# bertaveira/mojosplat

Hardware: AMD Instinct MI355X
Metric: frames/sec at 1M Gaussians 1920x1080 fwd; achieved HBM GB/s vs peak (higher is better)
Workload: dtype f32

## Files before the change

### mojosplat_amd/csrc/binning.hip

```cpp
#include <hip/hip_fp16.h>
#include <stdlib.h>
#include <string.h>

#include <algorithm>
#include <atomic>
#include <mutex>
#include <type_traits>
#include <vector>

#include "project_device.hpp"

#ifdef MS_DIAG
__device__ unsigned long long *g_diag_bin = nullptr;
#define MS_BIN_STAMP(k, j) do { if (g_diag_bin && threadIdx.x == 0 && blockIdx.x < 1024) g_diag_bin[((k) * 1024 + blockIdx.x) * 8 + (j)] = __builtin_amdgcn_s_memrealtime(); } while (0)
#else
#define MS_BIN_STAMP(k, j) do { } while (0)
#endif

namespace {

#ifndef MS_CHUNK
#define MS_CHUNK 2048
#endif
#ifndef MS_PH_WAVES
// ... 450 lines not shown
        unsigned long long bal[kSub];
        bool live[kSub];
        float p0[kSub], p1[kSub], p2[kSub], s0[kSub], s1[kSub], s2_[kSub];
#pragma unroll
        for (int k = 0; k < kSub; ++k) {
            const int64_t i = base + (int64_t)k * kHistThreads + threadIdx.x;
            live[k] = i < i1 && (!blocks || s_blk[(min(i, i1 - 1) >> block_shift) - blk0]);
            const int64_t j = live[k] ? i : i0;
            if constexpr (PREPARED) {
                const float4 r = cull[j];
                p0[k] = r.x; p1[k] = r.y; p2[k] = r.z; s0[k] = r.w; s1[k] = 0.f; s2_[k] = 0.f;
            } else {
                p0[k] = means3d[3 * j]; p1[k] = means3d[3 * j + 1]; p2[k] = means3d[3 * j + 2];
                s0[k] = scales[3 * j]; s1[k] = scales[3 * j + 1]; s2_[k] = scales[3 * j + 2];
            }
        }
#pragma unroll
        for (int k = 0; k < kSub; ++k) {
            keep[k] = false;
            {
                const float mx = V[0] * p0[k] + V[1] * p1[k] + V[2] * p2[k] + V[3];
                const float my = V[4] * p0[k] + V[5] * p1[k] + V[6] * p2[k] + V[7];
                const float z = V[8] * p0[k] + V[9] * p1[k] + V[10] * p2[k] + V[11];
                if (live[k] && !(z < P.near_plane || z > P.far_plane)) {
                    float sm = s0[k];
                    if constexpr (!PREPARED) {
                        sm = fmaxf(s0[k], fmaxf(s1[k], s2_[k]));
                        if (P.scales_are_log) sm = __expf(sm);
                    }
                    const float rz = __builtin_amdgcn_rcpf(z);
                    const float u = fminf(P.lim_x_pos, fmaxf(-P.lim_x_neg, mx * rz)), v = fminf(P.lim_y_pos, fmaxf(-P.lim_y_neg, my * rz));
                    const float s2 = lam * sm * sm;
                    const float fxz = P.fx * rz, fyz = P.fy * rz;
                    const float rx = 3.33f * __builtin_amdgcn_sqrtf(fxz * fxz * (1.0f + u * u) * s2 + P.eps2d) * 1.001f + 2.0f;
                    const float ry = 3.33f * __builtin_amdgcn_sqrtf(fyz * fyz * (1.0f + v * v) * s2 + P.eps2d) * 1.001f + 2.0f;
                    const float xs = P.fx * mx * rz + P.cx, ys = P.fy * my * rz + P.cy;
                    keep[k] = !(ys + ry < y_lo || ys - ry > y_hi || xs + rx < 0.f || xs - rx > P.W);
                }
            }
            bal[k] = __ballot(keep[k]);
        }
        uint32_t *sw = s_w[round & 1];
        ++round;
        if (lane == 0) {
#pragma unroll
            for (int k = 0; k < kSub; ++k) sw[k * 16 + w] = (uint32_t)__popcll(bal[k]);
        }
        __syncthreads();
#pragma unroll
        for (int k = 0; k < kSub; ++k) {
            uint32_t incl = lane < 16 ? sw[k * 16 + lane] : 0u;
#pragma unroll
            for (int d = 1; d < 16; d <<= 1) {
                const uint32_t o = (uint32_t)__shfl_up((int)incl, d);
                if (lane >= d) incl += o;
            }
            const int wu = __builtin_amdgcn_readfirstlane(w);
            const uint32_t total = (uint32_t)__builtin_amdgcn_readlane((int)incl, 15);
            const uint32_t before = written + (wu > 0 ? (uint32_t)__builtin_amdgcn_readlane((int)incl, wu - 1) : 0u);
            if (keep[k])
                seg[before + __builtin_amdgcn_mbcnt_hi((unsigned)(bal[k] >> 32), __builtin_amdgcn_mbcnt_lo((unsigned)bal[k], 0u))] =
                    (int32_t)(base + (int64_t)k * kHistThreads + threadIdx.x);
            written += total;
        }
    }
    if (threadIdx.x == 0) seg_count[blockIdx.x] = (int32_t)written;
    MS_BIN_STAMP(4, 2);
#ifdef MS_DIAG
    if (g_diag_bin && threadIdx.x == 0 && blockIdx.x < 1024) g_diag_bin[(4 * 1024 + blockIdx.x) * 8 + 3] = written;
#endif
}

template <bool PACK, int LEAN, bool CUT = false>
__global__ __launch_bounds__(kHistThreads, MS_PH_WAVES) void k_project_hist(
    int64_t N, const float *__restrict__ means3d, const float *__restrict__ scales,
    const float *__restrict__ quats, const float *__restrict__ opacities, const float *__restrict__ viewmat,
    ms::ProjParams P, Grid g, int64_t chunk, float *__restrict__ means2d, float *__restrict__ conics,
    float *__restrict__ depths, int32_t *__restrict__ radii, uint32_t *__restrict__ hist,
    uint32_t *__restrict__ wg_on_grid, unsigned long long *__restrict__ masks,
    const void *__restrict__ colors, int color_f16, float4 *__restrict__ rec, Candidates cand,
    LeanRec *__restrict__ lean, uint32_t *__restrict__ wg_depth, const uint32_t *__restrict__ tau,
    uint32_t *__restrict__ wg_far, uint32_t *__restrict__ has_far, uint32_t cut_stamp, LeanRec *__restrict__ near_recs,
    int keep_arrays, int64_t near_cap, unsigned int big_q_off, unsigned int big_q_cap,
    uint32_t *__restrict__ tile_total, unsigned long long *__restrict__ zero_flag, unsigned long long zero_stamp) {
    extern __shared__ uint32_t s_cnt[];
    const int T_local = (g.row_end - g.row_begin) * g.tw;
    unsigned int &s_on_grid = s_cnt[T_local];
    __shared__ unsigned int s_big_n;
    if (threadIdx.x == 0) s_big_n = 0;
    const BigQ bigq{reinterpret_cast<uint32_t *>(reinterpret_cast<char *>(s_cnt) + big_q_off), &s_big_n, big_q_cap};
    MS_BIN_STAMP(0, 0);
    __shared__ unsigned int s_near_n;
    __shared__ unsigned int s_next_slice;
    if (threadIdx.x == 0) { s_near_n = 0; s_next_slice = 0; }
    uint32_t *s_tau = s_cnt + T_local + 4;
    unsigned char *s_farflag = reinterpret_cast<unsigned char *>(s_tau + T_local);
    uint32_t far_pairs = 0;
    static_assert(!CUT || LEAN == 2, "depth-cut frames keep 12-byte box records");
    if constexpr (CUT)
        for (int t = threadIdx.x; t < T_local; t += kHistThreads) { s_tau[t] = tau[g.row_begin * g.tw + t]; s_farflag[t] = 0; }
    for (int t = threadIdx.x; t < T_local; t += kHistThreads) s_cnt[t] = 0;
    if (threadIdx.x == 0) { s_on_grid = 0; s_cnt[T_local + 1] = 0xffffffffu; s_cnt[T_local + 2] = 0u; s_cnt[T_local + 3] = 0u; }
    uint32_t dmin = 0xffffffffu, dmax = 0u;
    if (tile_total && blockIdx.x == 0) {
        for (int t = threadIdx.x; t < kClaimGroups * T_local; t += kHistThreads) __hip_atomic_store(&tile_total[t], 0u, __ATOMIC_RELAXED, __HIP_MEMORY_SCOPE_AGENT);
        asm volatile("s_waitcnt vmcnt(0)" ::: "memory");
    }
    __syncthreads();
    if (tile_total && blockIdx.x == 0 && threadIdx.x == 0)
        __hip_atomic_store(zero_flag, zero_stamp, __ATOMIC_RELEASE, __HIP_MEMORY_SCOPE_AGENT);
    __shared__ uint32_t s_pref[kMaxG + 1];
    CandMap map{s_pref};
    const int wg = chunk_of_block(blockIdx.x, gridDim.x);
    (void)chunk;
    int64_t i1 = N;
    if (cand.ids) {
        map.build(cand);
        i1 = (int64_t)s_pref[cand.n_segs];
    }
    const Deal deal(i1, wg, (int)gridDim.x);
    const uint32_t lane_u = threadIdx.x & 63u;
    auto count_plain = [&](int t, int64_t, int) __attribute__((always_inline)) { atomicAdd(&s_cnt[t], 1u); };
    auto count_cut = [&](int t, int64_t, int, uint32_t db) __attribute__((always_inline)) {
        if (db <= s_tau[t]) { atomicAdd(&s_cnt[t], 1u); dmin = min(dmin, db); dmax = max(dmax, db); }
        else { ++far_pairs; s_farflag[t] = 1; }
    };
    constexpr bool kTickets = kDeal == 64 && MS_PH_TICKETS != 0;
    const int n_slices = deal.iters * (kHistThreads / kDeal);
    for (int it = 0;; ++it) {
        int64_t base;
        if constexpr (kTickets) {
            int k = 0;
            if (lane_u == 0) k = (int)atomicAdd(&s_next_slice, 1u);
            k = __builtin_amdgcn_readfirstlane(k);
            if (k >= n_slices) break;
            base = ((int64_t)k * (int)gridDim.x + wg) * kDeal;
        } else {
            if (it >= deal.iters) break;
            base = deal.base(it);
        }
        const int64_t j = base + lane_u;
        int x0 = 0, x1 = 0, y0 = 0, y1 = 0, n = 0, edges = 0, gi = 0;
        bool on_grid = false;
        unsigned long long mask = ~0ull;
        uint32_t dbits_of_step = 0u;
        bool rec_pending = false;
        int64_t rec_b0 = 0;
        uint32_t rec_src = 0u;
        float rec_m0 = 0.f, rec_m1 = 0.f, rec_c0 = 0.f, rec_c1 = 0.f, rec_c2 = 0.f;
        auto write_record = [&](int64_t b0, uint32_t rec_src, float m0, float m1, float c0, float c1, float c2) __attribute__((always_inline)) {
            const float *opac_b = opacities ? opacities + b0 : nullptr;
            float col[3];
            if (color_f16) {
                const __half *c = reinterpret_cast<const __half *>(colors) + 3 * b0;
                col[0] = __half2float(c[3 * rec_src]); col[1] = __half2float(c[3 * rec_src + 1]); col[2] = __half2float(c[3 * rec_src + 2]);
            } else {
                const float *c = reinterpret_cast<const float *>(colors) + 3 * b0;
                const ms::F3 c3 = ms::ld_f32x3(c, rec_src);
                col[0] = c3.x; col[1] = c3.y; col[2] = c3.z;
            }
            const ms::RasterRecord r = ms::make_raster_record(m0, m1, c0, c1, c2, ms::ld_f32(opac_b, rec_src, 1, 0), col[0], col[1], col[2]);
            char *rb = reinterpret_cast<char *>(rec + 3 * base) + 48u * lane_u;
            *reinterpret_cast<float4 *>(rb) = r.a;
            *reinterpret_cast<float4 *>(rb + 16) = r.b;
            *reinterpret_cast<float4 *>(rb + 32) = r.c;
        };
        if (j < i1) {
            const bool gather = cand.ids != nullptr;
            const uint32_t src = gather ? (uint32_t)map.gaussian(cand, j) : lane_u;
            const int64_t b0 = gather ? 0 : base;
            const float *opac_b = opacities ? opacities + b0 : nullptr;
            const int64_t i = j;
            gi = (int)i;
            const ms::ProjOut o = ms::project_one<uint32_t, CUT>(src, means3d + 3 * b0, scales + 3 * b0, quats + 4 * b0, opac_b, viewmat, P);
            bool arrays = LEAN == 0;
            if constexpr (LEAN != 0) arrays = keep_arrays != 0;
            if (arrays) {
                reinterpret_cast<float2 *>(means2d)[i] = make_float2(o.m0, o.m1);
                conics[3 * i] = o.c0;
                conics[3 * i + 1] = o.c1;
                conics[3 * i + 2] = o.c2;
                depths[i] = o.d;
                reinterpret_cast<int2 *>(radii)[i] = make_int2(o.r0, o.r1);
            }
            if (rec && o.r0 > 0 && o.r1 > 0) {
                if constexpr (CUT) {
                    rec_pending = true;
                    rec_b0 = b0; rec_src = src;
                    rec_m0 = o.m0; rec_m1 = o.m1; rec_c0 = o.c0; rec_c1 = o.c1; rec_c2 = o.c2;
                } else {
                    write_record(b0, src, o.m0, o.m1, o.c0, o.c1, o.c2);
                }
            }
            if (o.r0 > 0 && o.r1 > 0) {
                on_grid = bin_box<PACK>(make_float2(o.m0, o.m1), make_int2(o.r0, o.r1), g, x0, x1, y0, y1, edges);
                n = (x1 - x0) * (y1 - y0);
                if (masks) {
                    if (LEAN == 2 && n > 32) mask = ~0ull;
                    else
                    if (PACK && n <= 16 && n > 0)
                        mask = clip_cells(reach_mask(o.m0, o.m1, o.c0, o.c1, o.c2, ms::ld_f32(opac_b, src, 1, 0), 2 * x0, 2 * x1,
                                                     2 * y0, 2 * y1, g.ts >> 1), edges, x1 - x0, y1 - y0);
                    else
                        mask = reach_mask(o.m0, o.m1, o.c0, o.c1, o.c2, ms::ld_f32(opac_b, src, 1, 0), x0, x1, y0, y1, g.ts);
                    if constexpr (LEAN != 2)
                        *reinterpret_cast<unsigned long long *>(reinterpret_cast<char *>(masks + base) + 8u * lane_u) = mask;
                }
            }
            dbits_of_step = __float_as_uint(o.d);
            if constexpr (LEAN != 0) {
                if (n > 0 && !CUT) { dmin = min(dmin, __float_as_uint(o.d)); dmax = max(dmax, __float_as_uint(o.d)); }
            }
            if constexpr (LEAN == 2 && !CUT) {
                uint32_t *q = reinterpret_cast<uint32_t *>(reinterpret_cast<char *>(reinterpret_cast<Lean12 *>(lean) + base) + 12u * lane_u);
                const uint32_t box = n > 0 ? ((uint32_t)x0 | ((uint32_t)y0 << 8) | ((uint32_t)(x1 - x0) << 16) | ((uint32_t)(y1 - y0) << 24)) : 0u;
                q[0] = box; q[1] = __float_as_uint(o.d); q[2] = (uint32_t)mask;
            }
            if constexpr (LEAN == 1)
                *reinterpret_cast<uint4 *>(reinterpret_cast<char *>(lean + base) + 16u * lane_u) = make_uint4((uint32_t)x0 | ((uint32_t)y0 << 16), (uint32_t)x1 | ((uint32_t)y1 << 16),
                                                                __float_as_uint(o.d), (uint32_t)n | ((uint32_t)edges << 28));
        }
        count_on_grid(on_grid, &s_on_grid);
        if constexpr (CUT) {
            uint32_t near32 = 0u;
            if (n > 0 && n <= kCoopThreshold) {
                const int w = x1 - x0;
                const float inv_w = __builtin_amdgcn_rcpf((float)w);
                unsigned int m = (unsigned int)mask & (n >= 32 ? 0xffffffffu : ((1u << n) - 1u));
                while (m) {
                    const int k = __ffs((int)m) - 1;
                    m &= m - 1;
                    const int r = (int)(((float)k + 0.5f) * inv_w);
                    const int t = (y0 + r - g.row_begin) * g.tw + x0 + (k - r * w);
                    if (dbits_of_step <= s_tau[t]) {
                        atomicAdd(&s_cnt[t], 1u);
                        near32 |= 1u << k;
                    } else {
                        ++far_pairs;
                        s_farflag[t] = 1;
                    }
                }
                if (near32) { dmin = min(dmin, dbits_of_step); dmax = max(dmax, dbits_of_step); }
            }
            walk_boxes<PACK>(gi, x0, x1, y0, y1, n > kCoopThreshold ? n : 0, edges, g, mask, count_cut, dbits_of_step, &bigq);
            const bool keep = near32 != 0u || n > kCoopThreshold;
            if (rec_pending && keep) write_record(rec_b0, rec_src, rec_m0, rec_m1, rec_c0, rec_c1, rec_c2);
            const unsigned long long kb = __ballot(keep);
            if (kb) {
                const int lane = threadIdx.x & 63;
                unsigned int wbase = 0;
                if (lane == 0) wbase = atomicAdd(&s_near_n, (unsigned int)__popcll(kb));
                wbase = (unsigned int)__builtin_amdgcn_readfirstlane((int)wbase);
                if (keep) {
                    const unsigned int pos = wbase + (unsigned int)__popcll(kb & ((1ull << lane) - 1ull));
                    const uint32_t box = (uint32_t)x0 | ((uint32_t)y0 << 8) | ((uint32_t)(x1 - x0) << 16) | ((uint32_t)(y1 - y0) << 24);
                    reinterpret_cast<uint4 *>(near_recs)[(int64_t)wg * near_cap + pos] = make_uint4(box, (uint32_t)gi, dbits_of_step, near32);
                }
            }
        } else {
            walk_boxes<PACK>(gi, x0, x1, y0, y1, n, edges, g, mask, count_plain, &bigq);
        }
    }
    if constexpr (CUT) drain_big_boxes<PACK, true>(bigq, g, count_cut);
    else drain_big_boxes<PACK, false>(bigq, g, count_plain);
    if constexpr (CUT) {
        {
#pragma unroll
            for (int d = 32; d > 0; d >>= 1) far_pairs += (uint32_t)__shfl_xor((int)far_pairs, d);
            if ((threadIdx.x & 63) == 0 && far_pairs) atomicAdd(&s_cnt[T_local + 3], far_pairs);
        }
    }
    if constexpr (LEAN != 0) {
        if (wg_depth) {
#pragma unroll
            for (int d = 32; d > 0; d >>= 1) {
                dmin = min(dmin, (uint32_t)__shfl_xor((int)dmin, d));
                dmax = max(dmax, (uint32_t)__shfl_xor((int)dmax, d));
            }
            if ((threadIdx.x & 63) == 0) { atomicMin(&s_cnt[T_local + 1], dmin); atomicMax(&s_cnt[T_local + 2], dmax); }
        }
    }
    MS_BIN_STAMP(0, 1);
    if (tile_total && threadIdx.x == 0) {
        while (__hip_atomic_load(zero_flag, __ATOMIC_ACQUIRE, __HIP_MEMORY_SCOPE_AGENT) != zero_stamp) __builtin_amdgcn_s_sleep(2);
    }
    __syncthreads();
    MS_BIN_STAMP(0, 2);
    uint32_t *row = hist + (size_t)wg * T_local;
    if (tile_total) {
        for (int t = threadIdx.x; t < T_local; t += kHistThreads) {
            const uint32_t c = s_cnt[t];
            row[t] = c ? __hip_atomic_fetch_add(&tile_total[(size_t)((blockIdx.x & 7) >> kClaimShift) * T_local + t], c, __ATOMIC_RELAXED, __HIP_MEMORY_SCOPE_AGENT) : 0u;
        }
    } else
    for (int t = threadIdx.x; t < T_local; t += kHistThreads) row[t] = s_cnt[t];
    if (threadIdx.x == 0) wg_on_grid[wg] = s_on_grid;
    if (threadIdx.x == 0 && blockIdx.x == 0) wg_on_grid[kMaxG] = 0;
    if constexpr (LEAN != 0) {
        if (wg_depth && threadIdx.x == 0) { wg_depth[2 * blockIdx.x] = s_cnt[T_local + 1]; wg_depth[2 * blockIdx.x + 1] = s_cnt[T_local + 2]; }
    }
    if constexpr (CUT) {
        {
            if (threadIdx.x == 0) { wg_far[wg] = s_cnt[T_local + 3]; wg_far[kMaxG + wg] = s_near_n; }
            for (int t = threadIdx.x; t < T_local; t += kHistThreads)
                if (s_farflag[t]) has_far[g.row_begin * g.tw + t] = cut_stamp;
        }
    }
    MS_BIN_STAMP(0, 3);
}

__global__ __launch_bounds__(kHistThreads) void k_isect_hist(
    int64_t N, const float *__restrict__ means2d, const int32_t *__restrict__ radii, Grid g,
    int64_t chunk, uint32_t *__restrict__ hist, int32_t *__restrict__ tiles_per_gauss,
    uint32_t *__restrict__ wg_on_grid) {
    extern __shared__ uint32_t s_cnt[];
    const int T_local = (g.row_end - g.row_begin) * g.tw;
    unsigned int &s_on_grid = s_cnt[T_local];
    for (int t = threadIdx.x; t < T_local; t += kHistThreads) s_cnt[t] = 0;
    if (threadIdx.x == 0) s_on_grid = 0;
    __syncthreads();
    const int wg = chunk_of_block(blockIdx.x, gridDim.x);
    (void)chunk;
    for_each_isect<false>(0, N, means2d, radii, nullptr, g, tiles_per_gauss, &s_on_grid, Candidates{nullptr, nullptr, 0, 0},
                   (int)gridDim.x, [&](int t, int64_t, int) { atomicAdd(&s_cnt[t], 1u); });
    __syncthreads();
    uint32_t *row = hist + (size_t)wg * T_local;
    for (int t = threadIdx.x; t < T_local; t += kHistThreads) row[t] = s_cnt[t];
    if (threadIdx.x == 0) wg_on_grid[wg] = s_on_grid;
    if (threadIdx.x == 0 && blockIdx.x == 0) wg_on_grid[kMaxG] = 0;
}

__device__ __forceinline__ int redo_signature(const Grid &g) { return (int)(0x80000000u | ((unsigned)g.tw & 0x7fffu) | (((unsigned)g.th & 0xffffu) << 15)); }

struct ScanTotalArgs {
    Grid g;
    const uint32_t *tile_count;
    int32_t *tile_ranges, *medium_list, *large_list, *xl_list;
    const uint32_t *wg_on_grid;
    int G;
    int32_t *redo_flag, *redo_count;
    int band_only;
    int64_t *info, *info_mirror;
    int32_t *order;
// ... 835 lines not shown
    const uint64_t k = src[start + e];
    flatten_ids[start + e] = (int32_t)(uint32_t)k;
    if (isect_ids) isect_ids[start + e] = ((int64_t)tile << 32) | (int64_t)(k >> 32);
}

__global__ __launch_bounds__(256) void k_offset_encode(int64_t M, const int64_t *__restrict__ ids,
                                                       int T, int32_t *__restrict__ offsets) {
    const int64_t idx = (int64_t)blockIdx.x * 256 + threadIdx.x;
    if (idx >= M) return;
    const int cur = (int)(ids[idx] >> 32);
    if (idx == 0)
        for (int t = 0; t <= cur && t < T; ++t) offsets[t] = 0;
    else {
        const int prev = (int)(ids[idx - 1] >> 32);
        for (int t = prev + 1; t <= cur && t < T; ++t) offsets[t] = (int32_t)idx;
    }
    if (idx == M - 1)
        for (int t = cur + 1; t < T; ++t) offsets[t] = (int32_t)M;
}

struct Plan {
    int G;
    int64_t chunk;
    int64_t near_cap;
    int T, T_local;
    size_t lds_bytes;
    size_t off_xtot;
    size_t off_hist, off_count, off_medium, off_large, off_xl, off_on_grid, off_mask, off_front, off_redo_flag,
        off_redo_list, off_redo_count, off_depth_wg, off_order, off_tau, off_has_far, off_wg_far, off_far_seg, off_cand_count, off_cand, off_lean, off_near, total;
};

bool make_plan(int64_t N, int tw, int th, int row_begin, int row_end, Plan &p) {
    p.T = tw * th;
    p.T_local = (row_end - row_begin) * tw;
    p.lds_bytes = (size_t)p.T_local * 4 + 16;
    int64_t G = ms::ceil_div(N > 0 ? N : 1, MS_CHUNK);
    if (G < 256) G = ms::ceil_div(N > 0 ? N : 1, kHistThreads) < 256 ? ms::ceil_div(N > 0 ? N : 1, kHistThreads) : 256;
    G = G < 1 ? 1 : (G > kMaxG ? kMaxG : G);
    if (p.lds_bytes > 64 * 1024 && G > 256) G = 256;
    p.chunk = ms::ceil_div(N > 0 ? N : 1, G);
    p.G = (int)ms::ceil_div(N > 0 ? N : 1, p.chunk);
    p.near_cap = ms::ceil_div(ms::ceil_div(N > 0 ? N : 1, (int64_t)kHistThreads), (int64_t)p.G) * kHistThreads;
    size_t o = 0;
    p.off_hist = o;   o += ms::align_up((size_t)kMaxG * p.T * 4, 256);
    p.off_count = o;  o += ms::align_up((size_t)p.T * 4, 256);
    p.off_xtot = o;   o += ms::align_up((size_t)8 * p.T * 4, 256);
    p.off_medium = o; o += ms::align_up((size_t)p.T * 4, 256);
    p.off_large = o;  o += ms::align_up((size_t)p.T * 4, 256);
    p.off_xl = o;     o += ms::align_up((size_t)p.T * 4, 256);
    p.off_on_grid = o; o += ms::align_up((size_t)kMaxG * 4 + 64, 256);
    p.off_front = o;      o += ms::align_up((size_t)p.T * 4, 256);
    p.off_redo_flag = o;  o += ms::align_up((size_t)p.T * 4, 256);
    p.off_redo_list = o;  o += ms::align_up((size_t)p.T * 4, 256);
    p.off_redo_count = o; o += 256;
    p.off_depth_wg = o;   o += ms::align_up((size_t)kMaxG * 8, 256);
    p.off_order = o;      o += ms::align_up((size_t)p.T * 4, 256);
    p.off_tau = o;        o += ms::align_up((size_t)p.T * 8, 256);
    p.off_has_far = o;    o += ms::align_up((size_t)p.T * 4, 256);
    p.off_wg_far = o;     o += ms::align_up((size_t)kMaxG * 8, 256);
    p.off_far_seg = o;    o += ms::align_up((size_t)p.T * 12, 256);
    p.off_cand_count = o; o += ms::align_up((size_t)kMaxG * 4, 256);
    p.off_mask = o;   o += ms::align_up((size_t)(N > 0 ? N : 1) * 8, 256);
    p.off_cand = o;   o += ms::align_up((size_t)(N > 0 ? N : 1) * 4, 256);
    p.off_lean = o;   o += ms::align_up((size_t)(N > 0 ? N : 1) * sizeof(LeanRec), 256);
    p.off_near = o;   o += ms::align_up((size_t)((N > 0 ? N : 1) + (int64_t)kHistThreads * (kMaxG + 1)) * sizeof(LeanRec), 256);
    p.total = o;
    return p.lds_bytes <= kMaxLds;
}

int check_grid(int tile_size, int tw, int th, int row_begin, int row_end) {
    MS_REQUIRE(tile_size > 0 && tw > 0 && th > 0, MS_ERR_INVALID_ARG, "isect: bad tile grid");
    MS_REQUIRE((int64_t)tw * th < (1ll << 30), MS_ERR_TOO_LARGE, "isect: tile grid too large");
    MS_REQUIRE(row_begin >= 0 && row_begin <= row_end && row_end <= th, MS_ERR_INVALID_ARG,
               "isect: bad row band [%d,%d) of %d", row_begin, row_end, th);
    return MS_OK;
}

unsigned int big_queue_cap(size_t used, int tile_w, int tile_h) {
    if (tile_w > 0xffff || tile_h > 0xffff || used >= kMaxLds) return 0u;
    const size_t room = (kMaxLds - used) / 32;
    return (unsigned int)(room < 256 ? room : 256);
}

template <class K>
int allow_big_lds(K kernel) {
    struct Seen { int dev; const void *fn; };
    static std::mutex mu;
    static std::vector<Seen> seen;
    const void *f = reinterpret_cast<const void *>(kernel);
    int dev = -1;
    MS_HIP(hipGetDevice(&dev));
    std::lock_guard<std::mutex> lock(mu);
    for (const Seen &e : seen)
        if (e.dev == dev && e.fn == f) return MS_OK;
    MS_HIP(hipFuncSetAttribute(f, hipFuncAttributeMaxDynamicSharedMemorySize, (int)kMaxLds));
    seen.push_back({dev, f});
    return MS_OK;
}

}

namespace {
int count_tail(const Plan &p, const Grid &g, char *ws, uint32_t *hist, uint32_t *count, int32_t *medium,
               int32_t *large, int32_t *xl, const uint32_t *wg_on_grid, int n_wg, int32_t *tile_ranges,
               int64_t *isect_info, int band_only, int64_t *info_mirror, hipStream_t stream, bool defer_total = false) {
    ScanTotalArgs A{g, count, tile_ranges, medium, large, xl, wg_on_grid, n_wg, (int32_t *)(ws + p.off_redo_flag),
                    (int32_t *)(ws + p.off_redo_count), band_only, isect_info, info_mirror, (int32_t *)(ws + p.off_order),
                    (uint32_t *)wg_on_grid + kMaxG, nullptr, nullptr, 0u, nullptr, 0, nullptr, nullptr};
    if (defer_total && p.T_local > 0) {
        A.ticket = nullptr;
        if (p.T_local <= 4096)
            hipLaunchKernelGGL(k_tile_scan_wg<16>, dim3((unsigned)ms::ceil_div(p.T_local, 16)), dim3(1024), 0, stream,
                               p.G, p.T_local, hist, count, A);
        else
            hipLaunchKernelGGL(k_tile_scan_wg<64>, dim3((unsigned)ms::ceil_div(p.T_local, 64)), dim3(1024), 0, stream,
                               p.G, p.T_local, hist, count, A);
        MS_LAUNCH_CHECK();
        return MS_OK;
    }
    if (p.T_local > 0) {
        if (p.T_local <= 4096)
            hipLaunchKernelGGL(k_tile_scan_wg<16>, dim3((unsigned)ms::ceil_div(p.T_local, 16)), dim3(1024), 0, stream,
                               p.G, p.T_local, hist, count, A);
        else {
            ScanTotalArgs A0 = A;
            A0.ticket = nullptr;
            hipLaunchKernelGGL(k_tile_scan_wg<64>, dim3((unsigned)ms::ceil_div(p.T_local, 64)), dim3(1024), 0, stream,
                               p.G, p.T_local, hist, count, A0);
            hipLaunchKernelGGL(k_tile_scan_total, dim3(1), dim3(1024), 0, stream, A0);
        }
    } else {
        A.ticket = nullptr;
        hipLaunchKernelGGL(k_tile_scan_total, dim3(1), dim3(1024), 0, stream, A);
    }
    MS_LAUNCH_CHECK();
    return MS_OK;
}
}

ms::FrontParams ms::front_params(int tile_size, int lazy, float depth_near, float depth_far, bool merged, bool split) {
    ms::FrontParams fp;
    fp.fixed_min = 0;
    fp.fixed_shift = -1;
    if (depth_near > 0.f && depth_far > depth_near) {
        uint32_t lo, hi;
        memcpy(&lo, &depth_near, 4);
        memcpy(&hi, &depth_far, 4);
        const uint32_t span = hi - lo;
        int bits = 0;
        while (bits < 32 && (span >> bits)) ++bits;
        fp.fixed_min = lo;
        fp.fixed_shift = bits > kFrontLogNB ? bits - kFrontLogNB : 0;
    }
    const int blocks_per_tile = ((tile_size + 15) / 16) * ((tile_size + 15) / 16);
    static const int front_env = [] { const char *e = getenv("MOJOSPLAT_FRONT_K"); return e ? atoi(e) : 0; }();
    int front_k = split ? 1280 : blocks_per_tile == 4 ? 1536 : min(kFrontK * blocks_per_tile, 2048);
    if (front_env >= 256 && front_env <= kFrontCap && blocks_per_tile > 1) front_k = front_env;
    fp.front_k = min(front_k << ((lazy >> 1) & 3), kFrontCap);
    fp.front_cap = merged ? min(kFrontCap, max(2048, (fp.front_k * 4 / 3 + 511) & ~511)) : kFrontCap;
    return fp;
}

void ms::isect_lazy_arrays(void *workspace, int64_t N, int tile_w, int tile_h, ms::LazyLists *out) {
    Plan p;
    make_plan(N, tile_w, tile_h, 0, tile_h, p);
    char *ws = (char *)workspace;
// ... 360 lines not shown
                                      int row_begin, int row_end, int tight, float *means2d, float *conics,
                                      float *depths,
                                      int32_t *radii, void *workspace, size_t workspace_bytes,
                                      int32_t *tile_ranges, int64_t *isect_info, int64_t *isect_info_mirror,
                                      void *stream_) {
    return ms::project_isect_count(N, means3d, scales, scales_are_log, quats, opacities, viewmat, fx, fy, cx, cy, W, H,
                                   eps2d, near_plane, far_plane, radius_clip, tile_size, row_begin, row_end, tight & 63,
                                   means2d, conics, depths, radii, workspace, workspace_bytes, tile_ranges, isect_info,
                                   isect_info_mirror, nullptr, 0, nullptr, stream_, 0u);
}

int ms::project_isect_count(int64_t N, const float *means3d, const float *scales, int scales_are_log,
                            const float *quats, const float *opacities, const float *viewmat,
                            float fx, float fy, float cx, float cy, int W, int H, float eps2d,
                            float near_plane, float far_plane, float radius_clip, int tile_size,
                            int row_begin, int row_end, int tight, float *means2d, float *conics,
                            float *depths,
                            int32_t *radii, void *workspace, size_t workspace_bytes,
                            int32_t *tile_ranges, int64_t *isect_info, int64_t *isect_info_mirror,
                            const void *colors3, int color_dtype, void *raster_records, void *stream_, uint32_t cut_stamp,
                            const float *block_bounds, int block_size) {
    hipStream_t stream = (hipStream_t)stream_;
    if (!opacities || !colors3) raster_records = nullptr;
    int block_shift = 0;
    if (block_bounds) {
        MS_REQUIRE(block_size >= 64 && (block_size & (block_size - 1)) == 0, MS_ERR_INVALID_ARG,
                   "project_isect_count: a prepared scene's block size must be a power of two >= 64 (got %d)", block_size);
        while ((1 << block_shift) < block_size) ++block_shift;
    }
    MS_REQUIRE(N >= 0 && W > 0 && H > 0 && tile_size > 0 && fx != 0.f && fy != 0.f, MS_ERR_INVALID_ARG,
               "project_isect_count: bad sizes / camera");
    const int tile_w = (W + tile_size - 1) / tile_size, tile_h = (H + tile_size - 1) / tile_size;
    if (int rc = check_grid(tile_size, tile_w, tile_h, row_begin, row_end)) return rc;
    MS_REQUIRE(workspace && tile_ranges && isect_info &&
                   (N == 0 || (means3d && scales && quats && viewmat && means2d && conics && depths && radii)),
               MS_ERR_INVALID_ARG, "project_isect_count: null pointer");
    MS_REQUIRE(((uintptr_t)quats & 15) == 0 && ((uintptr_t)means2d & 7) == 0 && ((uintptr_t)radii & 7) == 0 &&
                   ((uintptr_t)tile_ranges & 7) == 0,
               MS_ERR_INVALID_ARG, "project_isect_count: quats 16-byte, means2d/radii/tile_ranges 8-byte aligned");
    Plan p;
    const bool fits = make_plan(N, tile_w, tile_h, row_begin, row_end, p);
    MS_REQUIRE(fits, MS_ERR_TOO_LARGE, "project_isect_count: band of %d tiles needs %zu B of LDS (max %zu)",
               p.T_local, p.lds_bytes, kMaxLds);
    MS_REQUIRE(workspace_bytes >= p.total, MS_ERR_WORKSPACE, "project_isect_count: workspace %zu < %zu",
               workspace_bytes, p.total);
    char *ws = (char *)workspace;
    uint32_t *hist = (uint32_t *)(ws + p.off_hist);
    uint32_t *count = (uint32_t *)(ws + p.off_count);
    int32_t *medium = (int32_t *)(ws + p.off_medium);
    int32_t *large = (int32_t *)(ws + p.off_large), *xl = (int32_t *)(ws + p.off_xl);
    uint32_t *on_grid = (uint32_t *)(ws + p.off_on_grid);
    const bool pack = (tight & 4) && (tight & 1) && opacities && (tile_size & 1) == 0 && N < (1ll << 28);
    const Grid g{tile_size, tile_w, tile_h, row_begin, row_end, pack ? 1 : 0, 2 * tile_w - ((tight >> 3) & 1),
                 2 * tile_h - ((tight >> 4) & 1)};
    unsigned long long *masks = ((tight & 1) && opacities) ? (unsigned long long *)(ws + p.off_mask) : nullptr;
    const ms::ProjParams P = ms::make_proj_params(fx, fy, cx, cy, W, H, eps2d, near_plane, far_plane, radius_clip,
                                                  scales_are_log, opacities != nullptr);
    Candidates cand{nullptr, nullptr, 0, 0};
    if ((tight & kBandCull) && N >= (1ll << 28)) tight &= ~kBandCull;
    if ((tight & kBandCull) && N > 0) {
        int32_t *seg_count = (int32_t *)(ws + p.off_cand_count);
        hipLaunchKernelGGL(block_bounds ? k_band_precull<true> : k_band_precull<false>, dim3(p.G), dim3(kHistThreads), 0, stream, N,
                           means3d, scales, viewmat, P, (float)(row_begin * tile_size) - 1.0f, (float)(row_end * tile_size) + 1.0f,
                           p.chunk, (int32_t *)(ws + p.off_cand), seg_count, block_bounds, block_shift);
        MS_LAUNCH_CHECK();
        cand = Candidates{(const int32_t *)(ws + p.off_cand), seg_count, p.G, p.chunk};
    }
    static std::atomic<unsigned long long> claim_stamps{0x5ca1ab1e00000000ull};
    const bool claimed = (tight & ms::kTightClaimed) && (tight & kDeferTotal) && p.T_local > 0;
    {
        const bool lean = (tight & kLean) && raster_records && masks && tile_w <= 0xffff && tile_h <= 0xffff && N < (1ll << 28);
        const bool lean12 = lean && !pack && tile_w <= 255 && tile_h <= 255;
        auto kernel = pack ? (lean ? k_project_hist<true, 1> : k_project_hist<true, 0>)
                           : (lean12 ? (cut_stamp ? k_project_hist<false, 2, true> : k_project_hist<false, 2>)
                                     : lean ? k_project_hist<false, 1> : k_project_hist<false, 0>);
        const bool cut = cut_stamp != 0u;
        MS_REQUIRE(!cut || (lean12 && (tight & kDeferTotal)), MS_ERR_INVALID_ARG,
                   "project_isect_count: a depth-cut frame must be a lean sync-free frame on plain bins");
        size_t lds = p.lds_bytes + (cut ? (size_t)p.T_local * 5 + 16 : 0);
        MS_REQUIRE(lds <= kMaxLds, MS_ERR_TOO_LARGE, "project_isect_count: %d tiles with cut-offs need %zu B of LDS", p.T_local, lds);
        const unsigned int big_q_off = (unsigned int)ms::align_up(lds, 16);
        const unsigned int big_q_cap = big_queue_cap(big_q_off, tile_w, tile_h);
        lds = (size_t)big_q_off + (size_t)big_q_cap * 32;
        if (lds > 48 * 1024)
            if (int rc = allow_big_lds(kernel)) return rc;
        hipLaunchKernelGGL(kernel, dim3(p.G), dim3(kHistThreads), lds, stream, N, means3d, scales,
                           quats, opacities, viewmat, P, g, p.chunk, means2d, conics, depths, radii, hist, on_grid, masks,
                           colors3, color_dtype == MS_COLOR_F16 ? 1 : 0, (float4 *)raster_records, cand,
                           (LeanRec *)(ws + p.off_lean), (uint32_t *)(ws + p.off_depth_wg),
                           cut ? (const uint32_t *)(ws + p.off_tau) + (size_t)((tight >> 9) & 1) * p.T : nullptr, (uint32_t *)(ws + p.off_wg_far),
                           (uint32_t *)(ws + p.off_has_far), cut_stamp, (LeanRec *)(ws + p.off_near), (tight & ms::kTightKeepArrays) ? 1 : 0, p.near_cap,
                           big_q_off, big_q_cap, claimed ? (uint32_t *)(ws + p.off_xtot) : nullptr,
                           (unsigned long long *)(ws + p.off_redo_count + 64), claimed ? ++claim_stamps : 0ull);
        MS_LAUNCH_CHECK();
    }
    if (claimed) return MS_OK;
    return count_tail(p, g, ws, hist, count, medium, large, xl, on_grid, p.G, tile_ranges, isect_info,
                      (tight & 2) ? 1 : 0, isect_info_mirror, stream, (tight & kDeferTotal) != 0);
}

namespace {
int emit_impl(int64_t N, const float *means2d, const int32_t *radii, const float *depths, int tight, int lazy,
              float depth_near, float depth_far, int tile_size,
              int tile_w, int tile_h, int row_begin, int row_end, void *workspace, size_t workspace_bytes,
              const int32_t *tile_ranges, const int64_t *host_info, const int64_t *info_dev, int64_t cap,
              uint64_t *sort_keys, uint64_t *sort_tmp, int32_t *flatten_ids, int64_t *isect_ids,
              hipStream_t stream, const ms::BlockLists *blocks = nullptr, const ms::DeferredTotal *defer = nullptr) {
    const ms::BlockLists bl = blocks ? *blocks : ms::BlockLists{nullptr, nullptr, nullptr, 0, 0};
    const uint32_t cut_stamp = defer ? defer->cut_stamp : 0u;
    const int tau_out = (lazy >> 4) & 1;
    const bool write_tau = (lazy & 32) != 0;
    Plan p;
    const bool fits = make_plan(N, tile_w, tile_h, row_begin, row_end, p);
    MS_REQUIRE(fits, MS_ERR_TOO_LARGE, "isect_emit: band too large for LDS");
    MS_REQUIRE(workspace_bytes >= p.total, MS_ERR_WORKSPACE, "isect_emit: workspace %zu < %zu",
               workspace_bytes, p.total);
    char *ws = (char *)workspace;
    const uint32_t *hist = (const uint32_t *)(ws + p.off_hist);
    const int32_t *medium = (const int32_t *)(ws + p.off_medium);
    const int32_t *large = (const int32_t *)(ws + p.off_large), *xl = (const int32_t *)(ws + p.off_xl);
    const bool pack = (tight & 4) && (tight & 1) && (tile_size & 1) == 0 && N < (1ll << 28);
    const Grid g{tile_size, tile_w, tile_h, row_begin, row_end, pack ? 1 : 0, 2 * tile_w - ((tight >> 3) & 1),
                 2 * tile_h - ((tight >> 4) & 1)};
    const unsigned long long *masks = (tight & 1) ? (const unsigned long long *)(ws + p.off_mask) : nullptr;
    const bool spec = info_dev != nullptr;
    const int64_t max_count = spec ? 0 : host_info[1], n_medium = spec ? 0 : host_info[2],
                  n_large = spec ? 0 : host_info[3], n_xl = spec ? 0 : host_info[4];

    {
        const bool lean = (tight & kLean) && masks && tile_w <= 0xffff && tile_h <= 0xffff && N < (1ll << 28);
        const bool lean12 = lean && !pack && tile_w <= 255 && tile_h <= 255;
        const bool deferred = defer && p.T_local > 0;
        ScanTotalArgs A{};
        const uint32_t *xtot = (tight & ms::kTightClaimed) && p.T_local > 0 ? (const uint32_t *)(ws + p.off_xtot) : nullptr;
        A.xtot = xtot;
        if (deferred) {
            A = ScanTotalArgs{g, (const uint32_t *)(ws + p.off_count), const_cast<int32_t *>(tile_ranges), (int32_t *)(ws + p.off_medium),
                              (int32_t *)(ws + p.off_large), (int32_t *)(ws + p.off_xl), (const uint32_t *)(ws + p.off_on_grid), p.G,
                              (int32_t *)(ws + p.off_redo_flag), (int32_t *)(ws + p.off_redo_count), defer->band_only,
                              defer->info, defer->info_mirror, (int32_t *)(ws + p.off_order), nullptr,
                              nullptr, nullptr, 0u, nullptr, 0, nullptr, xtot};
            if (defer->cut_stamp) {
                MS_REQUIRE(lean12 && lazy, MS_ERR_INVALID_ARG, "isect emit: a depth-cut frame must be a lean, lazily sorted frame on plain bins");
                A.wg_far = (const uint32_t *)(ws + p.off_wg_far);
                A.tau = (const uint32_t *)(ws + p.off_tau) + (size_t)(1 - tau_out) * p.T;
                A.cut_stamp = defer->cut_stamp;
                A.far_zero = (uint32_t *)(ws + p.off_far_seg);
                A.near_recs = (const LeanRec *)(ws + p.off_near);
                A.near_cap = p.near_cap;
            }
        }
        size_t scatter_lds = p.lds_bytes + (A.cut_stamp ? (size_t)p.T_local * 4 + 16 : 0);
        const unsigned int big_q_off = (unsigned int)ms::align_up(scatter_lds, 16);
        const unsigned int big_q_cap = (lean ? big_queue_cap(big_q_off, tile_w, tile_h) : 0u);
        scatter_lds = (size_t)big_q_off + (size_t)big_q_cap * 32;
        auto pick = [&](auto packc, auto leanc) {
            constexpr bool PK = decltype(packc)::value;
            constexpr int LN = decltype(leanc)::value;
            return deferred ? k_isect_scatter<PK, LN, true> : k_isect_scatter<PK, LN, false>;
        };
        using I0 = std::integral_constant<int, 0>; using I1 = std::integral_constant<int, 1>; using I2 = std::integral_constant<int, 2>;
        auto kernel = pack ? (lean ? pick(std::true_type{}, I1{}) : pick(std::true_type{}, I0{}))
                           : (lean12 ? pick(std::false_type{}, I2{}) : lean ? pick(std::false_type{}, I1{}) : pick(std::false_type{}, I0{}));
        if (scatter_lds > 48 * 1024)
            if (int rc = allow_big_lds(kernel)) return rc;
        hipLaunchKernelGGL(kernel, dim3(p.G + (deferred ? 2 : 0)), dim3(kHistThreads), scatter_lds, stream, N, means2d, radii, depths, masks,
                           (const LeanRec *)(ws + p.off_lean), g, p.chunk, hist, tile_ranges, cap, sort_keys,
                           lazy && !lean ? (uint32_t *)(ws + p.off_depth_wg) : nullptr,
                           (tight & kBandCull) ? Candidates{(const int32_t *)(ws + p.off_cand), (const int32_t *)(ws + p.off_cand_count), p.G, p.chunk}
                                               : Candidates{nullptr, nullptr, 0, 0}, p.G, A, big_q_off, big_q_cap);
        MS_LAUNCH_CHECK();
        if (deferred && defer->sync_event) MS_HIP(hipEventRecord((hipEvent_t)defer->sync_event, stream));
    }

    static_assert(kSmallCap == kSmallCapDecl && kMediumCap == kMediumCapDecl && kLargeCap == kLargeCapDecl,
                  "sort class thresholds out of sync");
// ... 197 lines not shown
```

Before: 6236.

## Defer per-Gaussian reach-mask computation to an LDS queue drained by the whole block

In the lean 12-byte projection/histogram kernel, Gaussians that cover more than one tile no longer compute their tile reach mask inline. They are compacted with a ballot into an LDS queue holding their 2D mean, conic, opacity, box and index. After the main loop the whole block drains the queue, computing each mask, writing it to the lean record and counting tile hits. This targets lane divergence from the expensive reach_mask step, at the cost of extra LDS (up to about 76 KB total), one more barrier, and a lower occupancy ceiling.

```diff
diff --git a/mojosplat_amd/csrc/binning.hip b/mojosplat_amd/csrc/binning.hip
--- a/mojosplat_amd/csrc/binning.hip
+++ b/mojosplat_amd/csrc/binning.hip
@@ -556,13 +556,17 @@
     LeanRec *__restrict__ lean, uint32_t *__restrict__ wg_depth, const uint32_t *__restrict__ tau,
     uint32_t *__restrict__ wg_far, uint32_t *__restrict__ has_far, uint32_t cut_stamp, LeanRec *__restrict__ near_recs,
     int keep_arrays, int64_t near_cap, unsigned int big_q_off, unsigned int big_q_cap,
-    uint32_t *__restrict__ tile_total, unsigned long long *__restrict__ zero_flag, unsigned long long zero_stamp) {
+    uint32_t *__restrict__ tile_total, unsigned long long *__restrict__ zero_flag, unsigned long long zero_stamp,
+    unsigned int mask_q_off, unsigned int mask_q_cap) {
     extern __shared__ uint32_t s_cnt[];
     const int T_local = (g.row_end - g.row_begin) * g.tw;
     unsigned int &s_on_grid = s_cnt[T_local];
-    __shared__ unsigned int s_big_n;
-    if (threadIdx.x == 0) s_big_n = 0;
+    __shared__ unsigned int s_big_n, s_mq_n;
+    if (threadIdx.x == 0) { s_big_n = 0; s_mq_n = 0; }
     const BigQ bigq{reinterpret_cast<uint32_t *>(reinterpret_cast<char *>(s_cnt) + big_q_off), &s_big_n, big_q_cap};
+    constexpr bool kMaskQ = LEAN == 2 && !CUT && !PACK;
+    uint32_t *const mq = reinterpret_cast<uint32_t *>(reinterpret_cast<char *>(s_cnt) + mask_q_off);
+    const unsigned int mq_cap = kMaskQ ? mask_q_cap : 0u;
     MS_BIN_STAMP(0, 0);
     __shared__ unsigned int s_near_n;
     __shared__ unsigned int s_next_slice;
@@ -618,6 +622,8 @@
         bool on_grid = false;
         unsigned long long mask = ~0ull;
         uint32_t dbits_of_step = 0u;
+        bool defer = false;
+        float q_m0 = 0.f, q_m1 = 0.f, q_c0 = 0.f, q_c1 = 0.f, q_c2 = 0.f, q_op = 0.f;
         bool rec_pending = false;
         int64_t rec_b0 = 0;
         uint32_t rec_src = 0u;
@@ -672,6 +678,10 @@
                 if (masks) {
                     if (LEAN == 2 && n > 32) mask = ~0ull;
                     else
+                    if (kMaskQ && mq_cap) {
+                        q_m0 = o.m0; q_m1 = o.m1; q_c0 = o.c0; q_c1 = o.c1; q_c2 = o.c2; q_op = ms::ld_f32(opac_b, src, 1, 0);
+                        defer = n > 1 && o.c0 > 0.f && o.c2 > 0.f && q_op >= ms::kAlphaThreshold;
+                    } else
                     if (PACK && n <= 16 && n > 0)
                         mask = clip_cells(reach_mask(o.m0, o.m1, o.c0, o.c1, o.c2, ms::ld_f32(opac_b, src, 1, 0), 2 * x0, 2 * x1,
                                                      2 * y0, 2 * y1, g.ts >> 1), edges, x1 - x0, y1 - y0);
@@ -688,11 +698,42 @@
             if constexpr (LEAN == 2 && !CUT) {
                 uint32_t *q = reinterpret_cast<uint32_t *>(reinterpret_cast<char *>(reinterpret_cast<Lean12 *>(lean) + base) + 12u * lane_u);
                 const uint32_t box = n > 0 ? ((uint32_t)x0 | ((uint32_t)y0 << 8) | ((uint32_t)(x1 - x0) << 16) | ((uint32_t)(y1 - y0) << 24)) : 0u;
-                q[0] = box; q[1] = __float_as_uint(o.d); q[2] = (uint32_t)mask;
+                q[0] = box; q[1] = __float_as_uint(o.d);
+                if (!defer) q[2] = (uint32_t)mask;
             }
             if constexpr (LEAN == 1)
                 *reinterpret_cast<uint4 *>(reinterpret_cast<char *>(lean + base) + 16u * lane_u) = make_uint4((uint32_t)x0 | ((uint32_t)y0 << 16), (uint32_t)x1 | ((uint32_t)y1 << 16),
                                                                 __float_as_uint(o.d), (uint32_t)n | ((uint32_t)edges << 28));
+        }
+        if constexpr (kMaskQ) {
+            const unsigned long long qb = __ballot(defer);
+            if (qb) {
+                unsigned int qbase = 0;
+                if (lane_u == 0) qbase = atomicAdd(&s_mq_n, (unsigned int)__popcll(qb));
+                qbase = (unsigned int)__builtin_amdgcn_readfirstlane((int)qbase);
+                if (defer) {
+                    const unsigned int slot = qbase + __builtin_amdgcn_mbcnt_hi((unsigned)(qb >> 32), __builtin_amdgcn_mbcnt_lo((unsigned)qb, 0u));
+                    if (slot < mq_cap) {
+                        const uint32_t box = (uint32_t)x0 | ((uint32_t)y0 << 8) | ((uint32_t)(x1 - x0) << 16) | ((uint32_t)(y1 - y0) << 24);
+                        mq[slot] = __float_as_uint(q_m0); mq[mq_cap + slot] = __float_as_uint(q_m1);
+                        mq[2 * mq_cap + slot] = __float_as_uint(q_c0); mq[3 * mq_cap + slot] = __float_as_uint(q_c1);
+                        mq[4 * mq_cap + slot] = __float_as_uint(q_c2); mq[5 * mq_cap + slot] = __float_as_uint(q_op);
+                        mq[6 * mq_cap + slot] = box; mq[7 * mq_cap + slot] = (uint32_t)gi;
+                    } else {
+                        mask = reach_mask(q_m0, q_m1, q_c0, q_c1, q_c2, q_op, x0, x1, y0, y1, g.ts);
+                        reinterpret_cast<Lean12 *>(lean)[gi].mask32 = (uint32_t)mask;
+                        defer = false;
+                    }
+                }
+            }
+#ifdef MS_DIAG
+            if (g_diag_bin && blockIdx.x < 1024) {
+                const bool miss = masks && mq_cap && j < i1 && n > 0 && n <= 32 && !defer &&
+                                  mask != reach_mask(q_m0, q_m1, q_c0, q_c1, q_c2, q_op, x0, x1, y0, y1, g.ts);
+                const unsigned long long mb = __ballot(miss);
+                if (lane_u == 0 && mb) atomicAdd(&g_diag_bin[blockIdx.x * 8 + 4], (unsigned long long)__popcll(mb));
+            }
+#endif
         }
         count_on_grid(on_grid, &s_on_grid);
         if constexpr (CUT) {
@@ -732,7 +773,28 @@
                 }
             }
         } else {
-            walk_boxes<PACK>(gi, x0, x1, y0, y1, n, edges, g, mask, count_plain, &bigq);
+            walk_boxes<PACK>(gi, x0, x1, y0, y1, defer ? 0 : n, edges, g, mask, count_plain, &bigq);
+        }
+    }
+    if constexpr (kMaskQ) {
+        if (mq_cap) {
+            __syncthreads();
+            const unsigned int total = min(s_mq_n, mq_cap);
+            for (unsigned int e = threadIdx.x; e < total; e += kHistThreads) {
+                const float m0 = __uint_as_float(mq[e]), m1 = __uint_as_float(mq[mq_cap + e]);
+                const float c0 = __uint_as_float(mq[2 * mq_cap + e]), c1 = __uint_as_float(mq[3 * mq_cap + e]);
+                const float c2 = __uint_as_float(mq[4 * mq_cap + e]), op = __uint_as_float(mq[5 * mq_cap + e]);
+                const uint32_t box = mq[6 * mq_cap + e];
+                const int qi = (int)mq[7 * mq_cap + e];
+                const int bx0 = (int)(box & 0xffu), by0 = (int)((box >> 8) & 0xffu);
+                const int bx1 = bx0 + (int)((box >> 16) & 0xffu), by1 = by0 + (int)(box >> 24);
+                const unsigned long long m = reach_mask(m0, m1, c0, c1, c2, op, bx0, bx1, by0, by1, g.ts);
+                reinterpret_cast<Lean12 *>(lean)[qi].mask32 = (uint32_t)m;
+                walk_boxes<PACK>(qi, bx0, bx1, by0, by1, (bx1 - bx0) * (by1 - by0), 0, g, m, count_plain);
+            }
+#ifdef MS_DIAG
+            if (g_diag_bin && threadIdx.x == 0 && blockIdx.x < 1024) g_diag_bin[blockIdx.x * 8 + 5] = s_mq_n;
+#endif
         }
     }
     if constexpr (CUT) drain_big_boxes<PACK, true>(bigq, g, count_cut);
@@ -1734,6 +1796,13 @@
     return (unsigned int)(room < 256 ? room : 256);
 }
 
+constexpr size_t kPairLds = 80 * 1024 - 4096;
+unsigned int mask_queue_cap(size_t used) {
+    if (used >= kPairLds) return 0u;
+    const size_t room = (kPairLds - used) / 32;
+    return (unsigned int)(room < 2048 ? room : 2048);
+}
+
 template <class K>
 int allow_big_lds(K kernel) {
     struct Seen { int dev; const void *fn; };
@@ -2260,6 +2329,9 @@
         const unsigned int big_q_off = (unsigned int)ms::align_up(lds, 16);
         const unsigned int big_q_cap = big_queue_cap(big_q_off, tile_w, tile_h);
         lds = (size_t)big_q_off + (size_t)big_q_cap * 32;
+        const unsigned int mask_q_off = (unsigned int)ms::align_up(lds, 16);
+        const unsigned int mask_q_cap = lean12 && !cut ? mask_queue_cap(mask_q_off) : 0u;
+        lds = (size_t)mask_q_off + (size_t)mask_q_cap * 32;
         if (lds > 48 * 1024)
             if (int rc = allow_big_lds(kernel)) return rc;
         hipLaunchKernelGGL(kernel, dim3(p.G), dim3(kHistThreads), lds, stream, N, means3d, scales,
@@ -2269,7 +2341,7 @@
                            cut ? (const uint32_t *)(ws + p.off_tau) + (size_t)((tight >> 9) & 1) * p.T : nullptr, (uint32_t *)(ws + p.off_wg_far),
                            (uint32_t *)(ws + p.off_has_far), cut_stamp, (LeanRec *)(ws + p.off_near), (tight & ms::kTightKeepArrays) ? 1 : 0, p.near_cap,
                            big_q_off, big_q_cap, claimed ? (uint32_t *)(ws + p.off_xtot) : nullptr,
-                           (unsigned long long *)(ws + p.off_redo_count + 64), claimed ? ++claim_stamps : 0ull);
+                           (unsigned long long *)(ws + p.off_redo_count + 64), claimed ? ++claim_stamps : 0ull, mask_q_off, mask_q_cap);
         MS_LAUNCH_CHECK();
     }
     if (claimed) return MS_OK;
```

After: 6052, median of 6. 0.97x the previous value.
